# jandevaan/zzflate

Hardware: AMD Instinct MI355X
Metric: input GB/s compressed (whole node) + ratio, level 1, 1/2/4/8 MI355X (higher is better)
Workload: dtype u8; 1 GPU; 1024 MiB synthetic text per GPU (zz_generate_device kind=text, seed 0x5eed0002), level 1, zlib container, 32768-byte packets, input and output resident in HBM; level=1, packet_size=32768, bytes_per_gpu=1073741824, format=zlib, warm_window=0

## Files before the change

### zzflate_amd/csrc/zz_level1p.h

```cpp
#pragma once
#include "zz_level1.h"

namespace zz {

#define ZZ_L1P_THREADS (3 * ZZ_WAVE)
#ifndef ZZ_L1P_PRIO_W
#define ZZ_L1P_PRIO_W 3
#endif
#ifndef ZZ_L1P_PRIO_F
#define ZZ_L1P_PRIO_F 1
#endif
#ifndef ZZ_L1P_PRIO_E
#define ZZ_L1P_PRIO_E 0
#endif
#ifndef ZZ_L1P_ORDER_CHECK
#define ZZ_L1P_ORDER_CHECK 0
#endif
#ifndef ZZ_L1P_EXT32
#define ZZ_L1P_EXT32 0
#endif
#ifndef ZZ_L1P_ADLER3
#define ZZ_L1P_ADLER3 1
#endif
#ifndef ZZ_L1P_ADLER_U
#define ZZ_L1P_ADLER_U 6
#endif
#ifndef ZZ_L1P_LAZY_FLUSH
#define ZZ_L1P_LAZY_FLUSH 1
#endif
typedef __attribute__((address_space(3))) uint16_t lds_u16;

#define ZZ_L1P_NONE 64u
#define ZZ_L1P_SELF 65u
struct l1p_xch {
    uint32_t told[ZZ_WAVE + 4];
    uint8_t win[ZZ_WAVE + 4];
    uint16_t scal[ZZ_WAVE];
};



template <uint32_t BIAS>
__device__ __forceinline__ void l1p_parse(const zz_packet_params& P, const l1_pk& pk, uint16_t* T, uint32_t* tokbuf, l1p_xch* X, const uint32_t pw)
{
    const int lane = lane_id();
    const uint64_t below_me = (1ull << lane) - 1, above_me = ~((2ull << lane) - 1), self_bit = 1ull << lane;
    const uint32_t n = pk.n;
    const l1p_src SRC = l1p_make_src(P, pk.src, pk.end);
    const uint32_t NB = (n + ZZ_WAVE - 1) >> 6;
    lds_u32* const slot = (lds_u32*)tokbuf + lane + pw * ZZ_L1_TOKSLOT;
    uint64_t w = 0, w2 = 0;
    {
        const uint32_t p0 = pw * ZZ_WAVE + (uint32_t)lane;
        l1p_ld128<true>(SRC, p0 < n ? p0 : n - 1, w, w2);
    }
    ZZ_PROF_DECL
    uint32_t wmin = ZZ_WAVE;
    uint32_t mycout = 0;
    uint32_t hot_until = 0;
    if (pw == 1) l1_group_barrier();
    uint32_t xlo_next = pw ? 1u + BIAS : 0xFFFF0000u;
    for (uint32_t g = pw; g < NB; g += 2) {
        const uint32_t tag = (g + 1) << 16;
        const uint32_t xlo = xlo_next;
        xlo_next = (g << 6) + (2 * ZZ_WAVE - (ZZ_WAVE - 1)) + BIAS;
        if (mycout >= 2 * ZZ_WAVE) {
            const uint32_t p = (g << 6) + (uint32_t)lane;
            uint64_t wn = 0, wn2 = 0;
            if (g + 2 < NB) {
                const uint32_t pn = p + 2 * ZZ_WAVE;
                l1p_ld128<true>(SRC, pn < n ? pn : n - 1, wn, wn2);
            }
            l1_group_barrier();
            const uint32_t cin = uniform((uint32_t)X->scal[0]);
            mycout = cin > ZZ_WAVE ? cin - ZZ_WAVE : 0u;
            X->win[lane] = (uint8_t)ZZ_L1P_NONE;
            X->told[lane] = tag;
            X->scal[lane] = (uint16_t)mycout;
            l1_group_barrier();
            *slot = 0;
            w = wn;
            w2 = wn2;
            continue;
        }
        auto block = [&](auto interior_tag) {
            constexpr bool INT = decltype(interior_tag)::value;
            const uint32_t base = g << 6;
            const uint32_t p = base + (uint32_t)lane;
            const uint32_t nact = INT ? ZZ_WAVE : ((n - base) < ZZ_WAVE ? (n - base) : ZZ_WAVE);
            const bool active = INT ? true : lane < (int)nact;

            ZZ_T(6); ZZ_C(10, 1);
            const uint32_t h = calc_hash3((uint32_t)(w >> 8));
            const uint32_t oldraw = T[h];
            T[h] = (uint16_t)(p + 1 + BIAS);
            uint64_t wc, wc2;
            if (BIAS == 0) l1p_ld128<!INT>(SRC, __builtin_elementwise_sub_sat(oldraw, 1u), wc, wc2);
            else l1p_ld128<!INT>(SRC, (p + 1 + BIAS - oldraw > 0x8000u) ? 0 : (int32_t)(oldraw - 1u - BIAS), wc, wc2);
            uint64_t wn, wn2;
            if (!INT) { wn = 0; wn2 = 0; }
            if (INT || g + 2 < NB) {
                const uint32_t pn = p + 2 * ZZ_WAVE;
                l1p_ld128u<!INT>(SRC, INT ? pn : (pn < n ? pn : n - 1), wn, wn2);
            }
            ZZ_WAVE_SYNC();
            const uint32_t rb = T[h];
            const uint32_t qx = oldraw - xlo;
            const bool xd = active && qx < ZZ_WAVE;
#ifdef ZZ_L1P_X_NOCROSS
            const uint64_t XD = 0;
#else
            const uint64_t XD = ballot(xd);
#endif
            uint32_t talt;
            uint64_t wa, wa2;
            asm volatile("" : "=v"(talt), "=v"(wa), "=v"(wa2));
            const uint32_t qa = xd ? qx : ZZ_L1P_SELF;
            if (XD) {
                uint32_t v;
                do {
                    ZZ_C(13, 1);
                    v = *(volatile lds_u32*)&X->told[qa];
                } while (ballot((v >> 16) != g) & XD);
                talt = v & 0xFFFFu;
                if (xd) {
                    if (BIAS == 0) l1p_ld128<!INT>(SRC, __builtin_elementwise_sub_sat(talt, 1u), wa, wa2);
                    else l1p_ld128<!INT>(SRC, (p + 1 + BIAS - talt > 0x8000u) ? 0 : (int32_t)(talt - 1u - BIAS), wa, wa2);
                }
            }

            const uint64_t lostmask = ballot(active && rb != (uint32_t)(uint16_t)(p + 1 + BIAS));
            const uint32_t left = active ? n - p : 0;
            const uint32_t cap17 = INT ? 8u * (ZZ_WI_CAP + 1) : (left < ZZ_WI_CAP + 1 ? left : ZZ_WI_CAP + 1) << 3;
            uint64_t myset = self_bit;
            uint32_t infoB = 0;
            const uint32_t wraw = rb - 1u - BIAS - base;
            if (INT && ZZ_L1P_ORDER_CHECK) wmin = wraw < wmin ? wraw : wmin;
            if (lostmask) {
                uint32_t W = wraw;
                if (!INT && !active) W = (uint32_t)lane;
                if (!INT && active && wraw < wmin) wmin = wraw;
                myset = wave_match6(W);
                const uint64_t below = myset & below_me;
                const bool dup = below != 0 && active;
                const uint32_t ql = 63u - (uint32_t)__builtin_clzll(below | 1ull);
                const int qa = (int)(ql << 2);
                const uint64_t wq = ((uint64_t)(uint32_t)__builtin_amdgcn_ds_bpermute(qa, (int)(w >> 32)) << 32) | (uint32_t)__builtin_amdgcn_ds_bpermute(qa, (int)w);
                const uint64_t wq2 = ((uint64_t)(uint32_t)__builtin_amdgcn_ds_bpermute(qa, (int)(w2 >> 32)) << 32) | (uint32_t)__builtin_amdgcn_ds_bpermute(qa, (int)w2);
                const bool hard = (uint32_t)__builtin_popcountll(below) > 1u;
                uint32_t lbf;
                if (INT) {
                    lbf = (equal_bits128(w ^ wq, w2 ^ wq2, (((ZZ_WI_CAP << ZZ_WI_LENB_SHIFT) | ZZ_WI_EXTB) >> ZZ_WI_LENB_SHIFT) << 3) >> 3) << ZZ_WI_LENB_SHIFT;
                } else {
                    const uint32_t lb = equal_bits128(w ^ wq, w2 ^ wq2, cap17) >> 3;
                    lbf = lb > ZZ_WI_CAP ? ((ZZ_WI_CAP << ZZ_WI_LENB_SHIFT) | ZZ_WI_EXTB) : (lb << ZZ_WI_LENB_SHIFT);
                }
                const uint32_t di = ZZ_WI_DUP | (ql << ZZ_WI_QLANE_SHIFT) | (hard ? ZZ_WI_HARD : 0u) | lbf;
                infoB = dup ? di : 0u;
            }
            uint32_t ext;
            asm volatile("" : "=v"(ext));
            const bool gate = ZZ_L1P_EXT32 && BIAS == 0 && INT && g < hot_until;
            if (gate) {
                const bool all16 = ((w ^ wc) | (w2 ^ wc2)) == 0 && oldraw != 0;
                if (ballot(all16)) {
                    uint64_t ya, ya2, yc, yc2;
                    l1p_ld128u<false>(SRC, p + (all16 ? 16u : 0u), ya, ya2);
                    l1p_ld128u<false>(SRC, all16 ? oldraw + 15u : p, yc, yc2);
                    ext = equal_bits128(ya ^ yc, ya2 ^ yc2, 128u) >> 3;
                }
            }
            ZZ_T(0);
            l1_group_barrier();
            if (ZZ_L1P_PRIO_W != ZZ_L1P_PRIO_F) __builtin_amdgcn_s_setprio(ZZ_L1P_PRIO_W);
            ZZ_T(1);

            uint32_t cin;
            uint32_t told, info;
            uint64_t x;
            uint64_t MV;
            {
                const uint32_t sc = X->scal[0];
                const uint32_t r = X->win[qa];
                const bool moved = r != qa;
                const bool use3 = r == ZZ_L1P_NONE;
                const uint32_t toldh = (base - ZZ_WAVE + 1u + BIAS) + r;
                const uint32_t t1 = use3 ? talt : toldh;
                told = moved ? t1 : oldraw;
                ZZ_T(7);
                X->told[lane] = told | tag;
                MV = ballot(moved);
                const uint64_t LDM = MV & ~ballot(use3);
                constexpr uint32_t CAPA = (ZZ_WI_CAP | ZZ_WI_EXTA) << 3;
                auto compare = [&]() {
                    __builtin_amdgcn_sched_barrier(0);
                    const uint64_t c = use3 ? wa : wc, c2 = use3 ? wa2 : wc2;
                    x = w ^ c;
                    uint32_t la = equal_bits128(x, w2 ^ c2, INT ? CAPA : cap17) >> 3;
                    if (BIAS == 0 ? !told : (p + 1 + BIAS - told > 0x8000u)) la = 0;
                    info = infoB | (INT ? la : (la > ZZ_WI_CAP ? (ZZ_WI_CAP | ZZ_WI_EXTA) : la));
                };
                if (__builtin_expect(LDM == 0, 1)) {
                    compare();
                } else {
                    ZZ_C(14, 1);
                    uint64_t l0, l1;
                    if (BIAS == 0) l1p_ld128u<!INT>(SRC, __builtin_elementwise_sub_sat(told, 1u), l0, l1);
                    else l1p_ld128<!INT>(SRC, (p + 1 + BIAS - told > 0x8000u) ? 0 : (int32_t)(told - 1u - BIAS), l0, l1);
                    compare();
                    const uint64_t x3 = w ^ l0;
                    const uint32_t la3 = equal_bits128(x3, w2 ^ l1, INT ? CAPA : cap17) >> 3;
                    const uint32_t info3 = infoB | (INT ? la3 : (la3 > ZZ_WI_CAP ? (ZZ_WI_CAP | ZZ_WI_EXTA) : la3));
                    x = ((uint64_t)sel_lanes(LDM, (uint32_t)(x3 >> 32), (uint32_t)(x >> 32)) << 32) | sel_lanes(LDM, (uint32_t)x3, (uint32_t)x);
                    info = sel_lanes(LDM, info3, info);
                }
                cin = uniform(sc);
            }
            ZZ_T(8);
            const uint64_t E = ballot((info & (ZZ_WI_HARD | 0x1Cu | (0x1Cu << ZZ_WI_LENB_SHIFT))) != 0);
            {
                const uint32_t endl = (uint32_t)lane + (info & 31u);
                const uint64_t m = E >> (endl & 63u);
                const uint32_t nx = endl + (m ? (uint32_t)__builtin_ctzll(m) : 64u);
                info |= ((nx < 64u ? nx : 64u) & 63u) << ZZ_WI_NEXT_SHIFT;
            }

            ZZ_T(2); ZZ_C(12, (uint32_t)__builtin_popcountll(E)); ZZ_C(15, cin < 64 ? cin : 64);
            uint64_t mst = 0, usedB = 0;
            uint64_t cov;
            l1_walk_x Xw;
            Xw.hash = h; Xw.wlo = (uint32_t)w; Xw.whi = (uint32_t)(w >> 32); Xw.candbase = base + 1 + BIAS; Xw.hardok = INT ? 1u : 0u;
            asm volatile("" : "=v"(Xw.ovlen), "=v"(Xw.ovcand1));
            Xw.ovmL = 0; Xw.ovmC = 0;
            uint32_t& ovlen = Xw.ovlen; uint32_t& ovcand1 = Xw.ovcand1;
            uint64_t& ovmL = Xw.ovmL; uint64_t& ovmC = Xw.ovmC;
            uint32_t pos = cin;
            if (cin < ZZ_WAVE) {
                asm("s_bfm_b64 %0, %1, 0" : "=s"(cov) : "s"(cin));
                l1_fast_walk<true>(E, info, nact, pos, mst, cov, usedB, Xw);
            } else {
                cov = ~0ull;
            }
            while (pos < nact) {
                const int e = (int)pos;
                ZZ_C(11, 1);
                const uint64_t probed = ~cov | mst;
                const uint32_t inf = readlane(info, e);
                const uint32_t pe = base + (uint32_t)e;
                const uint32_t maxlen = (n - pe) < ZZ_MAX_LEN ? (n - pe) : ZZ_MAX_LEN;
                uint32_t mlen;
                if (!(inf & ZZ_WI_HARD)) {
                    const bool useB = (inf & ZZ_WI_DUP) && ((probed >> ZZ_WI_QLANE(inf)) & 1);
                    mlen = useB ? ZZ_WI_LENB(inf) : ZZ_WI_LENA(inf);
                    if (mlen >= 4) {
                        if (inf & (useB ? ZZ_WI_EXTB : ZZ_WI_EXTA)) {
                            const int32_t cand = useB ? (int32_t)(base + ZZ_WI_QLANE(inf)) : (int32_t)(readlane(told, e) - 1u - BIAS);
#ifdef ZZ_L1P_X_NOEXT
                            (void)cand;
                            mlen = maxlen < ZZ_WI_CAP ? maxlen : ZZ_WI_CAP;
#else
                            const uint32_t e16 = (gate && !useB && !((MV >> e) & 1)) ? readlane(ext, e) : 0xFFu;
                            if (e16 < 16u) mlen = 16u + e16;
                            else mlen = l1p_extend_match(SRC, pe, cand, maxlen, e16 == 16u ? 32u : ZZ_WI_CAP);
                            if (ZZ_L1P_EXT32) hot_until = g + 8u;
#endif
                            if (lane == e) ovlen = mlen | 0x8000u;
                            ovmL |= 1ull << e;
                        }
                        if (useB) usedB |= 1ull << e;
                    }
                } else {
                    const uint64_t S = readlane64(myset, e) & probed & ((1ull << e) - 1);
                    uint32_t cand1 = 0;
                    uint64_t xe = ~0ull;
                    if (S) {
                        const int c = 63 - __builtin_clzll(S);
                        cand1 = base + (uint32_t)c + 1 + BIAS;
                        xe = readlane64(w, e) ^ readlane64(w, c);
                    } else {
                        cand1 = readlane(told, e);
                        if (BIAS && pe + 1 + BIAS - cand1 > 0x8000u) cand1 = 0;
                        if (cand1) {
                            xe = readlane64(x, e);
                        }
                    }
                    mlen = 0;
                    if ((uint32_t)xe == 0 && maxlen >= 4) {
                        if (xe != 0) mlen = (uint32_t)__builtin_ctzll(xe) >> 3;
#ifdef ZZ_L1P_X_NOEXT
                        else mlen = 8;
#else
                        else mlen = l1p_extend_match(SRC, pe, (int32_t)(cand1 - 1u - BIAS), maxlen);
#endif
                        if (mlen > maxlen) mlen = maxlen;
                    }
                    if (lane == e) { ovlen = mlen | 0x8000u; ovcand1 = cand1; }
                    ovmL |= 1ull << e; ovmC |= 1ull << e;
                }
                if (mlen > 3) {
                    mst |= 1ull << e;
                    cov |= (mlen >= 64u - (uint32_t)e) ? (~0ull << e) : (((1ull << mlen) - 1) << e);
                    pos = (uint32_t)e + mlen;
                } else {
                    pos = (uint32_t)e + 1;
                }
                l1_fast_walk<false>(E, info, nact, pos, mst, cov, usedB, Xw);
            }
            ZZ_T(3);
            uint64_t committed;
            if (INT) {
                asm("s_orn2_b64 %0, %2, %1" : "=s"(committed) : "s"(cov), "s"(mst) : "scc");
            } else {
                uint32_t t;
                asm("s_min_u32 %1, %2, 64\n\ts_sub_u32 %1, 64, %1\n\ts_lshr_b64 %0, -1, %1\n\ts_andn2_b64 %0, %0, %3\n\ts_or_b64 %0, %0, %4"
                    : "=&s"(committed), "=&s"(t) : "s"(pos), "s"(cov), "s"(mst) : "scc");
            }
            {
                const uint64_t sv = myset & committed;
                const uint32_t fh = ffbh_or_ones((uint32_t)(sv >> 32)), fl = add_sat_k<32>(ffbh_or_ones((uint32_t)sv));
                X->win[lane] = (uint8_t)(63u - (fh < fl ? fh : fl));
                mycout = pos > ZZ_WAVE ? pos - ZZ_WAVE : 0u;
                X->scal[lane] = (uint16_t)mycout;
            }
            ZZ_T(4);
            l1_group_barrier();
            if (ZZ_L1P_PRIO_W != ZZ_L1P_PRIO_F) __builtin_amdgcn_s_setprio(ZZ_L1P_PRIO_F);
            ZZ_T(5);

            const uint32_t rb2 = T[h];
            {
                const uint32_t la_ = ZZ_WI_LENA(info) | 0x8000u, lb_ = ZZ_WI_LENB(info) | 0x8000u;
                const uint32_t tl = sel_lanes(ovmL, ovlen, sel_lanes(usedB, lb_, la_));
                const uint32_t cn = sel_lanes(ovmC, ovcand1, sel_lanes(usedB, base + ZZ_WI_QLANE(info) + 1 + BIAS, told));
                const uint32_t tmatch = (tl << 16) | (p + 1 + BIAS - cn);
                const uint32_t tlit = ZZ_TOK_LIT | (uint32_t)(w & 0xFF);
                *slot = keep_lanes(committed, sel_lanes(mst, tmatch, tlit));
            }
            const uint64_t INB = ballot((rb2 - (base + 1 + BIAS)) < ZZ_WAVE);
            const uint32_t taddr = (uint32_t)(uintptr_t)(__attribute__((address_space(3))) uint16_t*)(T + h);
            {
                const uint64_t rm = INB & ~committed;
                uint64_t saved;
                asm volatile("s_and_saveexec_b64 %0, %1\n\tds_write_b16 %2, %3\n\ts_mov_b64 exec, %0"
                             : "=&s"(saved) : "s"(rm), "v"(taddr), "v"(told) : "memory", "scc");
            }
            if (lostmask) {
                ZZ_WAVE_SYNC();
                const uint64_t wm = ballot((myset & committed & above_me) == 0) & committed & INB;
                uint64_t saved;
                asm volatile("s_and_saveexec_b64 %0, %1\n\tds_write_b16 %2, %3\n\ts_mov_b64 exec, %0"
                             : "=&s"(saved) : "s"(wm), "v"(taddr), "v"(p + 1 + BIAS) : "memory", "scc");
            }
            ZZ_WAVE_SYNC();
            w = wn;
            w2 = wn2;
        };
        if ((g << 6) + 3 * ZZ_WAVE + 15 <= n) block(std::true_type{});
        else block(std::false_type{});
    }
    if (((NB - 1) & 1u) != pw) l1_group_barrier();
    l1_group_barrier();
    if ((ballot(wmin < (uint32_t)lane) != 0 || P.dbg_viol) && lane == 0) atomicOr(P.err, ZZ_ERR_LDS_ORDER);
    ZZ_PROF_FLUSH_W(P, pw);
}

template <uint32_t BIAS>
__device__ __forceinline__ void l1p_packet_parser(const zz_packet_params& P, uint32_t k, uint16_t* T, uint32_t* tokbuf, l1p_xch* X, uint32_t pw)
{
    const int lane = lane_id();
    const l1_pk q = l1_packet_of(P, k);
    __builtin_amdgcn_s_setprio(ZZ_L1P_PRIO_F);
    uint4* t4 = (uint4*)T + pw * (ZZ_HASH_SIZE * sizeof(uint16_t) / 32);
    for (int i = lane; i < (int)(ZZ_HASH_SIZE * sizeof(uint16_t) / 32); i += ZZ_WAVE) t4[i] = make_uint4(0, 0, 0, 0);
    if (pw == 0) X->scal[lane] = 0;
    if (pw == 0) X->told[lane] = 0;
    if (pw == 1 && lane == 0) X->win[ZZ_L1P_SELF] = (uint8_t)ZZ_L1P_SELF;
    if (!BIAS && ZZ_L1P_ADLER3 && P.cks_kind == ZZ_CKS_ADLER) {
        uint32_t A = 0;
        uint64_t C = 0;
        wave_adler_part<ZZ_L1P_ADLER_U>(q.src, q.len, pw, 3, A, C);
        const uint64_t At = wave_sum64(A), Ct = wave_sum64(C);
        if (lane == 0) { uint64_t* part = (uint64_t*)(tokbuf + ZZ_L1_TOKSLOT) + 2 * pw; part[0] = At; part[1] = Ct; }
    }
    if (BIAS) {
        l1_group_barrier();
        if (pw == 0) {
            const uint64_t before = P.halo + q.off;
            uint32_t viol = 0;
            warm_prehash<BIAS, true>(T, q.src, (int32_t)(before < P.warm ? before : P.warm), q.end, 1, (uint32_t)(((uint16_t*)tokbuf + 255) - T), viol);
            if ((ballot(viol != 0) != 0 || P.dbg_viol) && lane == 0) atomicOr(P.err, ZZ_ERR_LDS_ORDER);
        }
    }
    l1_group_barrier();
    if (q.n > 0) {
        l1p_parse<BIAS>(P, q, T, tokbuf, X, pw);
    }
}

template <uint32_t BIAS>
__device__ __forceinline__ void l1p_packet_emitter(const zz_packet_params& P, uint32_t k, uint32_t* ring_words, const uint32_t* tokbuf)
{
    const int lane = lane_id();
    const l1_pk q = l1_packet_of(P, k);
    bitring ring;
    auto append_uniform = [&](uint32_t bits, uint32_t nbits) {
        if (ZZ_L1P_LAZY_FLUSH) ring_append_lazy(ring, lane == 0 ? bits : 0u, lane == 0 ? nbits : 0u);
        else ring_append_uniform(ring, bits, nbits);
    };
    if (ZZ_L1P_PRIO_E) __builtin_amdgcn_s_setprio(ZZ_L1P_PRIO_E);
    ZZ_PROF_DECL
    ring_init(ring, ring_words, q.out);
    const bool adler3 = !BIAS && ZZ_L1P_ADLER3 && P.cks_kind == ZZ_CKS_ADLER;
    uint64_t At = 0, Ct = 0;
    if (adler3) {
        uint32_t A = 0;
        uint64_t C = 0;
        wave_adler_part<ZZ_L1P_ADLER_U>(q.src, q.len, 2, 3, A, C);
        At = wave_sum64(A); Ct = wave_sum64(C);
    }
    if (BIAS) l1_group_barrier();
    else l1_group_barrier();
    ZZ_T(2);
    if (adler3) {
        if (lane == 0) {
            const uint64_t* part = (const uint64_t*)(tokbuf + ZZ_L1_TOKSLOT);
            At += part[0] + part[2]; Ct += part[1] + part[3];
            zz_cks c;
            c.a = (uint32_t)(At % ZZ_ADLER_MOD);
            c.b = (uint32_t)(((uint64_t)q.len * At - Ct) % ZZ_ADLER_MOD);
            P.cks[k] = c;
        }
    } else if (P.cks_kind == ZZ_CKS_ADLER) {
        zz_cks c = wave_adler(q.src, q.len);
        if (lane == 0) P.cks[k] = c;
    }
    ZZ_T(3);
    if (BIAS) l1_group_barrier();
    if (q.n > 0) {
        append_uniform((q.is_final ? 1u : 0u) | (1u << 1), 3);
        const uint32_t NB = (q.n + ZZ_WAVE - 1) >> 6;
        const lds_u32* slot = (const lds_u32*)tokbuf + lane;
        l1_group_barrier();
        ZZ_T(4);
        l1_group_barrier();
        ZZ_T(5); ZZ_C(11, 1);
        for (uint32_t g = 0; g < NB; ++g) {
            ZZ_T(1); ZZ_C(10, 1);
            l1_group_barrier();
            ZZ_T(0);
            const uint32_t tok = *slot;
            slot = lds_flip_slot((lds_u32*)slot);
#ifdef ZZ_L1P_X_NOEMIT
            if (g == 0)
#endif
#if ZZ_L1P_LAZY_FLUSH
            { uint32_t bits, nb; l1_token_bits(tok, bits, nb); ring_append_lazy(ring, bits, nb); }
#else
            l1_emit_tokens(ring, nullptr, tok);
#endif
        }
        append_uniform(0, 7);
    }
    if (!q.is_final) {
        append_uniform(0, 3);
        ring_pad_to_byte(ring);
        append_uniform(0xFFFE0001u, 32);
        append_uniform(q.src[q.len - 1], 8);
    } else if (q.n == 0) {
        append_uniform(1u | (1u << 1), 3);
        append_uniform(0, 7);
    }
    const uint32_t bytes = ZZ_L1P_LAZY_FLUSH ? ring_finish_lazy(ring) : ring_finish(ring);
    if (lane == 0) {
        P.sizes[k] = bytes;
        if (bytes > P.slot_stride) atomicOr(P.err, ZZ_ERR_SLOT_OVERFLOW);
    }
    ZZ_T(6);
    ZZ_PROF_FLUSH_W(P, 2);
}

__global__ __launch_bounds__(ZZ_L1P_THREADS) void k_encode_l1p(zz_packet_params P)
{
    __shared__ uint16_t T[ZZ_HASH_SIZE];
    __shared__ uint32_t ring_words[ZZ_RING_WORDS];
    __shared__ __attribute__((aligned(512))) uint32_t tokbuf[2 * ZZ_L1_TOKSLOT];
    __shared__ l1p_xch X;
    const uint32_t k = blockIdx.x;
    const uint32_t wv = uniform(threadIdx.x >> 6);
    if (wv < 2) l1p_packet_parser<0u>(P, k, T, tokbuf, &X, wv);
    else l1p_packet_emitter<0u>(P, k, ring_words, tokbuf);
}
__global__ __launch_bounds__(ZZ_L1P_THREADS) void k_encode_l1pw(zz_packet_params P)
{
    __shared__ uint16_t T[ZZ_HASH_SIZE];
    __shared__ uint32_t ring_words[ZZ_RING_WORDS];
    __shared__ __attribute__((aligned(512))) uint32_t tokbuf[2 * ZZ_L1_TOKSLOT];
    __shared__ l1p_xch X;
    const uint32_t k = blockIdx.x;
    const uint32_t wv = uniform(threadIdx.x >> 6);
    if (wv < 2) l1p_packet_parser<32768u>(P, k, T, tokbuf, &X, wv);
    else l1p_packet_emitter<32768u>(P, k, ring_words, tokbuf);
}

}
```

### zzflate_amd/csrc/zz_wave.h

```cpp
#pragma once
#include "zz_common.h"

namespace zz {

#define ZZ_WAVE_SYNC()                                              \
    do {                                                            \
        __builtin_amdgcn_fence(__ATOMIC_SEQ_CST, "wavefront");      \
        __builtin_amdgcn_wave_barrier();                            \
    } while (0)

__device__ __forceinline__ uint64_t ballot(bool p) { return __builtin_amdgcn_ballot_w64(p); }
__device__ __forceinline__ int lane_id() { return (int)(threadIdx.x & 63); }

__device__ __forceinline__ uint32_t readlane(uint32_t v, int l)
{
    return (uint32_t)__builtin_amdgcn_readlane((int)v, __builtin_amdgcn_readfirstlane(l));
}
__device__ __forceinline__ uint64_t readlane64(uint64_t v, int l)
{
    uint32_t lo = readlane((uint32_t)v, l), hi = readlane((uint32_t)(v >> 32), l);
    return ((uint64_t)hi << 32) | lo;
}
__device__ __forceinline__ uint32_t uniform(uint32_t v) { return (uint32_t)__builtin_amdgcn_readfirstlane((int)v); }

#define ZZ_DPP_ROW_SHR(n) (0x110 + (n))
#define ZZ_DPP_ROW_BCAST15 0x142
#define ZZ_DPP_ROW_BCAST31 0x143

__device__ __forceinline__ uint32_t wave_scan_incl(uint32_t x)
{
    int v = (int)x;
    v += __builtin_amdgcn_update_dpp(0, v, ZZ_DPP_ROW_SHR(1), 0xf, 0xf, false);
    v += __builtin_amdgcn_update_dpp(0, v, ZZ_DPP_ROW_SHR(2), 0xf, 0xf, false);
    v += __builtin_amdgcn_update_dpp(0, v, ZZ_DPP_ROW_SHR(4), 0xf, 0xf, false);
    v += __builtin_amdgcn_update_dpp(0, v, ZZ_DPP_ROW_SHR(8), 0xf, 0xf, false);
    v += __builtin_amdgcn_update_dpp(0, v, ZZ_DPP_ROW_BCAST15, 0xa, 0xf, false);
    v += __builtin_amdgcn_update_dpp(0, v, ZZ_DPP_ROW_BCAST31, 0xc, 0xf, false);
    return (uint32_t)v;
}

__device__ __forceinline__ uint32_t wave_sum(uint32_t x)
{
    return readlane(wave_scan_incl(x), 63);
}
__device__ __forceinline__ uint64_t wave_sum64(uint64_t x)
{
#pragma unroll
    for (int o = 32; o >= 1; o >>= 1) x += __shfl_xor(x, o);
    return x;
}

__device__ __forceinline__ uint64_t wave_match6(uint32_t key)
{
    uint32_t m0, m1, m2, m3, m4, m5;
    uint64_t b0, b1, b2, b3, b4, b5;
    asm("v_bfe_i32 %0, %12, 0, 1\n\tv_bfe_i32 %1, %12, 1, 1\n\tv_bfe_i32 %2, %12, 2, 1\n\t"
        "v_bfe_i32 %3, %12, 3, 1\n\tv_bfe_i32 %4, %12, 4, 1\n\tv_bfe_i32 %5, %12, 5, 1\n\t"
        "v_cmp_ne_u32_e64 %6, 0, %0\n\tv_cmp_ne_u32_e64 %7, 0, %1\n\tv_cmp_ne_u32_e64 %8, 0, %2\n\t"
        "v_cmp_ne_u32_e64 %9, 0, %3\n\tv_cmp_ne_u32_e64 %10, 0, %4\n\tv_cmp_ne_u32_e64 %11, 0, %5\n\t"
        "s_nop 1"
        : "=&v"(m0), "=&v"(m1), "=&v"(m2), "=&v"(m3), "=&v"(m4), "=&v"(m5),
          "=&s"(b0), "=&s"(b1), "=&s"(b2), "=&s"(b3), "=&s"(b4), "=&s"(b5)
        : "v"(key));
    uint32_t lo, hi;
    lo = __builtin_amdgcn_bitop3_b32((uint32_t)b0, m0, ~0u, 0x82);
    hi = __builtin_amdgcn_bitop3_b32((uint32_t)(b0 >> 32), m0, ~0u, 0x82);
    lo = __builtin_amdgcn_bitop3_b32((uint32_t)b1, m1, lo, 0x82); hi = __builtin_amdgcn_bitop3_b32((uint32_t)(b1 >> 32), m1, hi, 0x82);
    lo = __builtin_amdgcn_bitop3_b32((uint32_t)b2, m2, lo, 0x82); hi = __builtin_amdgcn_bitop3_b32((uint32_t)(b2 >> 32), m2, hi, 0x82);
    lo = __builtin_amdgcn_bitop3_b32((uint32_t)b3, m3, lo, 0x82); hi = __builtin_amdgcn_bitop3_b32((uint32_t)(b3 >> 32), m3, hi, 0x82);
    lo = __builtin_amdgcn_bitop3_b32((uint32_t)b4, m4, lo, 0x82); hi = __builtin_amdgcn_bitop3_b32((uint32_t)(b4 >> 32), m4, hi, 0x82);
    lo = __builtin_amdgcn_bitop3_b32((uint32_t)b5, m5, lo, 0x82); hi = __builtin_amdgcn_bitop3_b32((uint32_t)(b5 >> 32), m5, hi, 0x82);
    return ((uint64_t)hi << 32) | lo;
}

template <int NB> __device__ __forceinline__ uint64_t wave_match_bits(uint32_t key)
{
    uint32_t lo = ~0u, hi = ~0u;
#pragma unroll
    for (int b = 0; b < NB; ++b) {
        const uint32_t m = (uint32_t)((int32_t)(key << (31 - b)) >> 31);
        const uint64_t B = ballot(m != 0);
        lo = __builtin_amdgcn_bitop3_b32((uint32_t)B, m, lo, 0x82);
        hi = __builtin_amdgcn_bitop3_b32((uint32_t)(B >> 32), m, hi, 0x82);
    }
    return ((uint64_t)hi << 32) | lo;
}

__device__ __forceinline__ uint32_t sel_lanes(uint64_t m, uint32_t a, uint32_t b)
{
    uint32_t r;
    asm("v_cndmask_b32_e64 %0, %1, %2, %3" : "=v"(r) : "v"(b), "v"(a), "s"(m));
    return r;
}
__device__ __forceinline__ uint32_t keep_lanes(uint64_t m, uint32_t a)
{
    uint32_t r;
    asm("v_cndmask_b32_e64 %0, 0, %1, %2" : "=v"(r) : "v"(a), "s"(m));
    return r;
}

__device__ __forceinline__ uint64_t load64(const uint8_t* p)
{
    uint64_t v;
    __builtin_memcpy(&v, p, 8);
    return v;
}
__device__ __forceinline__ uint32_t load32(const uint8_t* p)
{
    uint32_t v;
    __builtin_memcpy(&v, p, 4);
    return v;
}
__device__ __forceinline__ uint64_t load64_safe(const uint8_t* p, const uint8_t* end)
{
    if (p + 8 <= end) return load64(p);
    uint64_t v = 0;
    for (int i = 0; i < 8; ++i)
        if (p + i < end) v |= (uint64_t)p[i] << (8 * i);
    return v;
}
__device__ __forceinline__ uint32_t load32_safe(const uint8_t* p, const uint8_t* end)
{
    if (p + 4 <= end) return load32(p);
    uint32_t v = 0;
    for (int i = 0; i < 4; ++i)
        if (p + i < end) v |= (uint32_t)p[i] << (8 * i);
    return v;
}

__device__ __forceinline__ void coop_copy(uint8_t* dst, const uint8_t* src, uint64_t n, uint32_t tid,
                                          uint32_t nthreads)
{
    if (n == 0) return;
    uint64_t head = (16 - ((uintptr_t)dst & 15)) & 15;
    if (head > n) head = n;
    if (tid < head) dst[tid] = src[tid];
    uint64_t body = (n - head) >> 4;
    const uint8_t* s = src + head;
    uint4* d = (uint4*)(dst + head);
    uint64_t i = tid;
    for (; i + 3 * (uint64_t)nthreads < body; i += 4 * (uint64_t)nthreads) {
        uint4 v0, v1, v2, v3;
        __builtin_memcpy(&v0, s + (i << 4), 16);
        __builtin_memcpy(&v1, s + ((i + nthreads) << 4), 16);
        __builtin_memcpy(&v2, s + ((i + 2 * (uint64_t)nthreads) << 4), 16);
        __builtin_memcpy(&v3, s + ((i + 3 * (uint64_t)nthreads) << 4), 16);
        d[i] = v0; d[i + nthreads] = v1; d[i + 2 * (uint64_t)nthreads] = v2; d[i + 3 * (uint64_t)nthreads] = v3;
    }
    for (; i < body; i += nthreads) {
        uint4 v;
        __builtin_memcpy(&v, s + (i << 4), 16);
        d[i] = v;
    }
    uint64_t done = head + (body << 4);
    uint64_t tail = n - done;
    if (tid < tail) dst[done + tid] = src[done + tid];
}

}
```

Baseline: 144.0 GB/s.

## Compact sparse token lanes into full waves before Huffman emission

The emit loop now ballots the non-zero tokens in each 64-token group and packs them with ds_permute into a carry register. A wave-wide emit call runs only once a full wave of real tokens has gathered, plus one flush at the end. This is meant to cut the number of emit and bit-packing passes when many slots hold empty tokens, for example where literals have been merged into matches. The cost is extra ballot, popcount, permute and select work per group, and it assumes zero tokens emit no bits.

Measured after the change: 144.9 GB/s, median of 6. Within noise of the previous version (+0.6%).

```diff
diff --git a/zzflate_amd/csrc/zz_level1p.h b/zzflate_amd/csrc/zz_level1p.h
--- a/zzflate_amd/csrc/zz_level1p.h
+++ b/zzflate_amd/csrc/zz_level1p.h
@@ -444,6 +444,14 @@
         ZZ_T(4);
         l1_group_barrier();
         ZZ_T(5); ZZ_C(11, 1);
+        auto code = [&](uint32_t t) {
+#if ZZ_L1P_LAZY_FLUSH
+            uint32_t bits, nb; l1_token_bits(t, bits, nb); ring_append_lazy(ring, bits, nb);
+#else
+            l1_emit_tokens(ring, nullptr, t);
+#endif
+        };
+        uint32_t H = 0, h = 0;
         for (uint32_t g = 0; g < NB; ++g) {
             ZZ_T(1); ZZ_C(10, 1);
             l1_group_barrier();
@@ -451,14 +459,29 @@
             const uint32_t tok = *slot;
             slot = lds_flip_slot((lds_u32*)slot);
 #ifdef ZZ_L1P_X_NOEMIT
-            if (g == 0)
-#endif
-#if ZZ_L1P_LAZY_FLUSH
-            { uint32_t bits, nb; l1_token_bits(tok, bits, nb); ring_append_lazy(ring, bits, nb); }
+            (void)tok; (void)H;
 #else
-            l1_emit_tokens(ring, nullptr, tok);
+            const uint64_t M = ballot(tok != 0);
+            const uint32_t c = (uint32_t)__builtin_popcountll(M);
+            uint32_t R = tok, J = tok;
+            if (h | (c ^ ZZ_WAVE)) {
+                if (c == 0) continue;
+                const uint32_t rank = wave_rank(M);
+                const uint32_t to = tok ? rank : c + (uint32_t)lane - rank;
+                R = (uint32_t)__builtin_amdgcn_ds_permute((int)((h + to) << 2), (int)tok);
+                J = sel_lanes(~0ull << h, R, H);
+            }
+            if (h + c >= ZZ_WAVE) {
+                code(J);
+                H = R;
+                h = h + c - ZZ_WAVE;
+            } else {
+                H = J;
+                h += c;
+            }
 #endif
         }
+        if (h) code(keep_lanes((1ull << h) - 1, H));
         append_uniform(0, 7);
     }
     if (!q.is_final) {
diff --git a/zzflate_amd/csrc/zz_wave.h b/zzflate_amd/csrc/zz_wave.h
--- a/zzflate_amd/csrc/zz_wave.h
+++ b/zzflate_amd/csrc/zz_wave.h
@@ -71,6 +71,11 @@
     lo = __builtin_amdgcn_bitop3_b32((uint32_t)b4, m4, lo, 0x82); hi = __builtin_amdgcn_bitop3_b32((uint32_t)(b4 >> 32), m4, hi, 0x82);
     lo = __builtin_amdgcn_bitop3_b32((uint32_t)b5, m5, lo, 0x82); hi = __builtin_amdgcn_bitop3_b32((uint32_t)(b5 >> 32), m5, hi, 0x82);
     return ((uint64_t)hi << 32) | lo;
+}
+
+__device__ __forceinline__ uint32_t wave_rank(uint64_t m)
+{
+    return __builtin_amdgcn_mbcnt_hi((uint32_t)(m >> 32), __builtin_amdgcn_mbcnt_lo((uint32_t)m, 0u));
 }
 
 template <int NB> __device__ __forceinline__ uint64_t wave_match_bits(uint32_t key)
```
